# MILVLG/mmnas

Measured on AMD Instinct MI355X. Metric: supernet fwd+bwd steps/sec (VQA arch, bs=64), higher is better.
Workload: dtype f32 (bf16x6 split-operand MFMA, fp32 accumulate); 1 GPU; Net_Search supernet WEIGHT step: sample + fwd + BCE(sum) + bwd (+ gradient all-reduce), HSIZE 256, B=64/GPU, 100x2048 regions + 14 tokens, dropout 0.1 (search_vqa.py:279-292; BASELINE configs[2]); global_batch=64, parallelism=dp1, grad_allreduce=none, rccl_ranks=1, rank_id_sum_ok=True, lstm_fallback=False, dp_rows=1, dp_buckets=3, optimizer_in_step=False, gemm_split=6, hip_force_dev_kernarg=1

## Files before the change

include/mmnas_hip.h:

```cpp
#ifndef MMNAS_HIP_H
#define MMNAS_HIP_H

#include <stddef.h>
#include <stdint.h>

#ifdef __cplusplus
extern "C" {
#endif

#define MMNAS_ABI_VERSION 1

enum {
  MMNAS_OK = 0,
  MMNAS_E_SHAPE = -1,
  MMNAS_E_ARG = -2,
  MMNAS_E_LAUNCH = -3
};

enum {
  MMNAS_F_NORM = 1,
  MMNAS_F_RESIDUAL = 2,
  MMNAS_F_MASK = 4,
  MMNAS_F_REL = 8,
  MMNAS_F_SELF = 16,
// ... 156 lines not shown
size_t mmnas_rel_fused_bwd_ws_floats(int B, int Sq, int Sk);
int mmnas_rel_fused_bwd(const float* raw, const float* Wy, const float* by, const float* Wr,
                        const float* br, const float* dbiasT, float* dWy, float* dby, float* dWr,
                        float* dbr, float* ws, int B, int Sq, int Sk, int C, int R, int H,
                        void* stream);
int mmnas_rel_fused_fwd_ragged(const float* raw, const float* Wy, const float* by, const float* Wr, const float* br,
                               float* biasT, int B, int S, int C, int R, int H, const int* off, void* stream);
int mmnas_rel_fused_bwd_ragged(const float* raw, const float* Wy, const float* by, const float* Wr, const float* br,
                               const float* dbiasT, float* dWy, float* dby, float* dWr, float* dbr, float* ws,
                               int B, int S, int C, int R, int H, const int* off, const int* tile_off, int ntiles, void* stream);

#define MMNAS_REL_MULTI_MAX 32
typedef struct mmnas_rel_multi {
  int B, S, C, R, H, n_ops;
  const float* raw;
  const float* Wy; const float* by;
  float* dWy; float* dby;
  const float* Wr[MMNAS_REL_MULTI_MAX];
  const float* br[MMNAS_REL_MULTI_MAX];
  float* biasT[MMNAS_REL_MULTI_MAX];
  const float* dbiasT[MMNAS_REL_MULTI_MAX];
  float* dWr[MMNAS_REL_MULTI_MAX]; float* dbr[MMNAS_REL_MULTI_MAX];
  const int* off; const int* tile_off; int ntiles, reserved;
  float* ws;
  const unsigned char* key_mask;
} mmnas_rel_multi;
int mmnas_rel_multi_supported(int C, int R, int H);
size_t mmnas_rel_multi_bwd_ws_floats(int B, int S);
int mmnas_rel_multi_fwd(const mmnas_rel_multi* m, void* stream);
int mmnas_rel_multi_bwd(const mmnas_rel_multi* m, void* stream);
int mmnas_set_rel_hoist(int on);
int mmnas_set_rel_keylimit(int on);
int mmnas_set_guided_hoist(int on);
int mmnas_set_rel_overlap(int on);

typedef struct mmnas_mha_desc {
  int B, H, Sq, Sk, dh;
  int ldq, ldk, ldv, ldo;
  const float* Q; const float* K; const float* V;
  const uint8_t* mask;
  const float* biasT;
  float* O;
  float* lse;
  float drop_p; uint32_t drop_site; uint64_t drop_seed;
  const float* dO;
  float* dQ; float* dK; float* dV;
  float* dbiasT;
  float* delta;
  const int* q_off; const int* k_off;
} mmnas_mha_desc;

int mmnas_mha_core_fwd(const mmnas_mha_desc* d, void* stream);
int mmnas_mha_core_bwd(const mmnas_mha_desc* d, void* stream);
int mmnas_mha_core_fwd_indexed(const mmnas_mha_desc* d, const int* kv_idx, void* stream);

typedef struct mmnas_att_op {
  int B, Sq, Sk, d, di, H, dh, R;
  int flags;
  float drop_p, eps;
  uint64_t seed;
  const float* xq;
  const float* xkv;
  const uint8_t* mask;
  const float* rel;
  const float* Wq; const float* Wk; const float* Wv;
  const float* Wm;
  const float* Wr; const float* br;
  const float* ln_a; const float* ln_b;
  float* y;
  void* save;
  void* ws;
  const float* dy;
  float* dxq;
  float* dxkv;
  float* drel;
  float* dWq; float* dWk; float* dWv; float* dWm;
  float* dWr; float* dbr; float* dln_a; float* dln_b;
  int C;
  const float* Wy; const float* by;
  float* dWy; float* dby;
  const int* q_off; const int* k_off;
  int Mq, Mk;
  const int* rel_tile_off;
  int rel_ntiles, reserved2;
} mmnas_att_op;

typedef struct mmnas_plan {
  size_t save_bytes, ws_fwd_bytes, ws_bwd_bytes;
} mmnas_plan;

int mmnas_set_small_ops(int on);
int mmnas_set_small_bwd(int on);
int mmnas_set_small_ffn(int on);
int mmnas_att_op_plan(const mmnas_att_op* op, mmnas_plan* plan);
int mmnas_att_op_fwd(const mmnas_att_op* op, void* stream);
int mmnas_att_op_bwd(const mmnas_att_op* op, void* stream);

typedef struct mmnas_mlp_op {
  int M, nl;
  int dims[4];
  int flags;
  float drop_p, eps;
  uint64_t seed;
  const float* x;
  const float* W[3];
  const float* b[3];
// ... 150 lines not shown
```

mmnas_amd/_lib.py:

```python
import ctypes as C
import logging
import os

import torch

from . import switches

_HERE = os.path.dirname(os.path.abspath(__file__))
LIB_PATH = os.environ.get(switches.LIB_PATH.name) or os.path.join(_HERE, 'lib', 'libmmnas_hip.so')

log = logging.getLogger('mmnas_amd')


def _launch_configuration():
    name = 'HIP_FORCE_DEV_KERNARG'
    if name in os.environ:
        return os.environ[name], 'inherited'
    if torch.cuda.is_initialized():
        log.warning('mmnas_amd was imported after HIP had initialised and %s is not set: kernel arguments go through host-visible '
                    'memory, the ~300 short launches of a step run 20-40 %% slower.  Export %s=1 or import mmnas / mmnas_amd '
                    'before the first CUDA call.', name, name)
        return None, 'unset_after_hip_init'
    os.environ[name] = '1'
    return '1', 'set_by_library'
# ... 138 lines not shown
    'mmnas_layernorm_bwd': (_i, [_fp, _fp, _fp, _fp, _fp, _fp, _fp, _fp, _fp, _f, _u64, _u32, _i, _i, _f, _fp]),
    'mmnas_layernorm_bwd_ws_floats': (_sz, [_i, _i]),
    'mmnas_colsum': (_i, [_fp, _fp, _i, _i, _i, _fp]),
    'mmnas_eltwise_fwd': (_i, [_i, _fp, _fp, _sz, _fp]),
    'mmnas_eltwise_bwd': (_i, [_i, _fp, _fp, _fp, _sz, _fp]),
    'mmnas_drop_add': (_i, [_fp, _fp, _fp, _sz, _f, _u64, _u32, _fp]),
    'mmnas_glu_fwd': (_i, [_fp, _fp, _i, _i, _i, _f, _u64, _u32, _fp]),
    'mmnas_glu_bwd': (_i, [_fp, _fp, _fp, _i, _i, _i, _f, _u64, _u32, _fp]),
    'mmnas_rel_bias_fwd': (_i, [_fp, _fp, _fp, _fp, _i, _i, _i, _i, _i, _fp]),
    'mmnas_rel_bias_bwd': (_i, [_fp, _fp, _fp, _fp, _fp, _fp, _fp, _i, _i, _i, _i, _i, _i, _fp]),
    'mmnas_row_is_zero': (_i, [_fp, _fp, C.c_long, _i, _fp]),
    'mmnas_glimpse1_supported': (_i, [_i]),
    'mmnas_glimpse1_bwd_ws_floats': (_sz, [C.c_long, _i]),
    'mmnas_glimpse1_fwd': (_i, [_fp, _fp, _fp, _fp, C.c_long, _i, _fp]),
    'mmnas_glimpse1_bwd': (_i, [_fp, _fp, _fp, _fp, _fp, _fp, _fp, C.c_long, _i, _fp]),
    'mmnas_attflat_pool_fwd': (_i, [_fp, _fp, _fp, _fp, _fp, _i, _i, _i, _i, _fp]),
    'mmnas_attflat_pool_bwd': (_i, [_fp, _fp, _fp, _fp, _fp, _fp, _i, _i, _i, _i, _fp]),
    'mmnas_relation_embedding': (_i, [_fp, _fp, _fp, _i, _i, _fp]),
    'mmnas_semantic_embedding': (_i, [_fp, _fp, _fp, _fp, _i, _i, _i, C.c_long, _fp]),
    'mmnas_onehot_rows': (_i, [_fp, _i, _i, C.POINTER(C.c_int), _fp]),
    'mmnas_mixed_sum_ws_floats': (_sz, []),
    'mmnas_mixed_sum_fwd': (_i, [C.POINTER(_fp), _i, _fp, _fp, _sz, _fp]),
    'mmnas_mixed_sum_bwd': (_i, [C.POINTER(_fp), _i, _fp, _fp, _fp, _i, _fp, _fp, _sz, _fp]),
    'mmnas_alpha_full_step': (_i, [_fp, _fp, _fp, _fp, _fp, _i, _i, _f, _f, _f, _f, _i, _fp]),
    'mmnas_alpha_full_step_wd': (_i, [_fp, _fp, _fp, _fp, _fp, _i, _i, _f, _f, _f, _f, _f, _i, _fp]),
    'mmnas_alpha_two_step': (_i, [_fp, _fp, _fp, _fp, _fp, _i, _i, C.POINTER(C.c_int), _f, _f, _f, _f, _f, _i, _fp]),
    'mmnas_alpha_full_step_cost': (_i, [_fp] * 7 + [_i, _i, _f, _f, _f, _f, _f, _f, _f, _i, _i, _fp]),
    'mmnas_alpha_two_step_cost': (_i, [_fp] * 7 + [_i, _i, C.POINTER(C.c_int), _f, _f, _f, _f, _f, _f, _f, _i, _i, _fp]),
    'mmnas_embedding_bwd': (_i, [_fp, _fp, _fp, C.c_long, _i, C.c_long, _fp]),
    'mmnas_node_mix_fwd': (_i, [_fp, _fp, _fp, _i, _fp, _fp, _i, _i, _f, _fp]),
    'mmnas_node_mix_bwd': (_i, [_fp, _fp, _fp, _i, _fp, _fp, _fp, _i, _fp, _fp, _i, _i, _f, _fp]),
    'mmnas_node_mix_bwd_ln': (_i, [_fp, _fp, _fp, _i, _fp, _fp, _i, _fp, _fp, _fp, _fp, _fp, _fp, _fp, _fp, _f, _u64, _u32, _i, _i, _f, _fp]),
    'mmnas_embedding_bwd_det': (_i, [_fp, _fp, _fp, _fp, C.c_long, _i, C.c_long, _f, _fp]),
    'mmnas_embedding_bwd_det_ws_floats': (_sz, [C.c_long, _i]),
    'mmnas_rel_fused_supported': (_i, [_i, _i, _i]),
    'mmnas_rel_fused_fwd': (_i, [_fp, _fp, _fp, _fp, _fp, _fp, _i, _i, _i, _i, _i, _i, _fp]),
    'mmnas_rel_fused_bwd_ws_floats': (_sz, [_i, _i, _i]),
    'mmnas_rel_fused_bwd': (_i, [_fp, _fp, _fp, _fp, _fp, _fp, _fp, _fp, _fp, _fp, _fp, _i, _i, _i, _i, _i, _i, _fp]),
    'mmnas_rel_fused_fwd_ragged': (_i, [_fp, _fp, _fp, _fp, _fp, _fp, _i, _i, _i, _i, _i, _fp, _fp]),
    'mmnas_rel_fused_bwd_ragged': (_i, [_fp] * 11 + [_i, _i, _i, _i, _i, _fp, _fp, _i, _fp]),
    'mmnas_rel_multi_supported': (_i, [_i, _i, _i]),
    'mmnas_rel_multi_bwd_ws_floats': (_sz, [_i, _i]),
    'mmnas_rel_multi_fwd': (_i, [C.POINTER(RelMulti), _fp]),
    'mmnas_rel_multi_bwd': (_i, [C.POINTER(RelMulti), _fp]),
    'mmnas_set_rel_hoist': (_i, [_i]),
    'mmnas_set_rel_keylimit': (_i, [_i]),
    'mmnas_set_wgrad_live': (_i, [_i]),
    'mmnas_wgrad_live_table_ints': (_i, [_i]),
    'mmnas_wgrad_live_table': (_i, [_fp, _fp, _i, _i, _fp, _fp]),
    'mmnas_set_guided_hoist': (_i, [_i]),
    'mmnas_set_rel_overlap': (_i, [_i]),
    'mmnas_mha_core_fwd': (_i, [C.POINTER(MhaDesc), _fp]),
    'mmnas_mha_core_bwd': (_i, [C.POINTER(MhaDesc), _fp]),
    'mmnas_mha_core_fwd_indexed': (_i, [C.POINTER(MhaDesc), _fp, _fp]),
    'mmnas_itm_pair_head': (_i, [_fp] * 11 + [C.c_long, _i, _i, _f, _fp]),
    'mmnas_rank_matrix': (_i, [_fp, _i, _i, C.c_long, _fp, _fp, _fp, _fp, _fp, _fp]),
    'mmnas_row_topk': (_i, [_fp, _i, _i, C.c_long, _i, _fp, _fp, _fp]),
    'mmnas_vgd_targets': (_i, [_fp, _fp, _fp, _i, _i, C.c_double, _i, _fp, _fp, _fp, _fp, _fp, _fp, _fp]),
    'mmnas_vgd_ground': (_i, [_fp] * 5 + [_i, _i, C.c_double] + [_fp] * 7),
    'mmnas_vqa_answer': (_i, [_fp, _i, _i, C.c_long, _fp, C.c_long, _i, _i] + [_fp] * 4 + [_i] + [_fp] * 5),
    'mmnas_vqa_accuracy': (_i, [_fp] * 4 + [_i] * 4 + [_fp, _fp, _fp]),
    'mmnas_vqa_answer_targets': (_i, [_fp, _i, _i, _i, _fp, _fp, _fp]),
    'mmnas_vgd_loss_fwd': (_i, [_fp] * 6 + [_i] * 6 + [C.c_double, C.c_double] + [_fp] * 5),
    'mmnas_itm_triplet_loss_fwd': (_i, [_fp, _fp, _fp, C.c_long, _i, _f, _i, _fp, _fp, _fp]),
    'mmnas_loss_grad_scale': (_i, [_fp, _fp, _fp, _sz, _fp]),
    'mmnas_vgd_head_supported': (_i, [_i, _i]),
    'mmnas_vgd_head_bwd_ws_floats': (_sz, [_i, _i, _i]),
    'mmnas_vgd_head_fwd': (_i, [_fp] * 12 + [_i, _i, _i, _f, _i, _fp]),
    'mmnas_vgd_head_bwd': (_i, [_fp] * 20 + [_i, _i, _i, _f, _i, _fp]),
    'mmnas_att_op_plan': (_i, [C.POINTER(AttOp), C.POINTER(Plan)]),
    'mmnas_att_op_fwd': (_i, [C.POINTER(AttOp), _fp]),
    'mmnas_att_op_bwd': (_i, [C.POINTER(AttOp), _fp]),
    'mmnas_mlp_op_plan': (_i, [C.POINTER(MlpOp), C.POINTER(Plan)]),
    'mmnas_mlp_op_fwd': (_i, [C.POINTER(MlpOp), _fp]),
    'mmnas_mlp_op_bwd': (_i, [C.POINTER(MlpOp), _fp]),
    'mmnas_chain_plan': (_i, [C.POINTER(Chain), C.POINTER(C.c_size_t)]),
    'mmnas_chain_fwd': (_i, [C.POINTER(Chain), _fp]),
    'mmnas_chain_bwd': (_i, [C.POINTER(Chain), _fp]),
    'mmnas_chain_join': (_i, [_fp, _fp]),
    'mmnas_head_plan': (_i, [C.POINTER(Head), C.POINTER(C.c_size_t)]),
    'mmnas_head_fwd': (_i, [C.POINTER(Head), _fp]),
    'mmnas_head_bwd': (_i, [C.POINTER(Head), _fp]),
    'mmnas_bce_logits_sum_fwd': (_i, [_fp, _fp, _fp, _sz, _fp]),
    'mmnas_bce_logits_bwd': (_i, [_fp, _fp, _fp, _fp, _sz, _fp]),
    'mmnas_im2col_seq': (_i, [_fp, _fp, _i, _i, _i, _i, _fp]),
    'mmnas_pack_rows': (_i, [_fp, _fp, _fp, _i, _i, _i, _fp]),
    'mmnas_unpack_rows': (_i, [_fp, _fp, _fp, _i, _i, _i, _fp]),
    'mmnas_pad_seq': (_i, [_fp, _fp, _i, _i, _i, _i, _i, C.c_long, _fp]),
    'mmnas_col2im_seq': (_i, [_fp, _fp, _i, _i, _i, _i, _fp]),
    'mmnas_dwconv_seq_fwd': (_i, [_fp, _fp, _fp, _fp, _i, _i, _i, _i, _fp]),
    'mmnas_dwconv_seq_bwd': (_i, [_fp, _fp, _fp, _fp, _fp, _fp, _i, _i, _i, _i, _fp]),
    'mmnas_pack_segments': (_i, [_fp, _i, _fp, _f, _i, _fp]),
    'mmnas_pack_segments_host': (_i, [C.POINTER(Segment), _i, _fp, _f, _i, _fp]),
    'mmnas_adam_step': (_i, [_fp, _fp, _fp, _fp, _sz, _f, _f, _f, _f, _f, _fp, _f, _i, _fp]),
    'mmnas_sgd_step': (_i, [_fp, _fp, _fp, _sz, _f, _f, _f, _f, _i, _i, _fp, _f, _fp]),
    'mmnas_sumsq': (_i, [_fp, _sz, _fp, _fp]),
    'mmnas_prof_enable': (_i, [_i]),
    'mmnas_prof_collect': (_i, [C.POINTER(ProfStat)]),
}

_lib = None


class MMNasHipError(RuntimeError):
    pass

# ... 44 lines not shown
```

mmnas_amd/csrc/attention.hip:

```cpp
#include <string.h>
#include "common.h"

namespace mmnas {

struct MhaK {
  int B, H, Sq, Sk, dh, nch;
  int ldq, ldk, ldv, ldo;
  const float* Q; const float* K; const float* V;
  const uint8_t* mask; const float* biasT;
  float* O; float* stats;
  DropCfg drop; float scale;
  const float* dO; float* dQ; float* dK; float* dV; float* dbiasT; float* delta;
  const int* qoff; const int* koff;
};

template <int ROWS, int DHC, int NT>
struct TileRegs { float4 v[(ROWS * (DHC / 4) + NT - 1) / NT]; };

template <int ROWS, int DHC, int NT>
__device__ __forceinline__ void tile_fetch(TileRegs<ROWS, DHC, NT>& t, const float* __restrict__ src, int nvalid,
                                           int ld, int tid) {
  constexpr int F4 = DHC / 4, N = (ROWS * F4 + NT - 1) / NT;
#pragma unroll
  for (int i = 0; i < N; ++i) {
// ... 978 lines not shown
      if (s + 1 < NSTEP) P1(32 * ((w + s + 1) % NKB), tA[nxt], tD[nxt], tb[nxt], tm[nxt]);
      P2(k0, tA[cur], tD[cur], tb[cur], tm[cur]);
      if (s + 1 < NSTEP) {
#pragma unroll
        for (int i = 0; i < 64; ++i) {
          __builtin_amdgcn_sched_group_barrier(0x008, 1, 0);
          __builtin_amdgcn_sched_group_barrier(0x002, MMNAS_MHA_VPM, 0);
        }
      }
      P34(k0, cp, tA[cur], tD[cur]);
    }
    __syncthreads();
  }
  if (active) {
#pragma unroll
    for (int jc = 0; jc < JC; ++jc) {
      const int col = 32 * jc + l31;
#pragma unroll
      for (int r = 0; r < 16; ++r) {
        const int q = q0 + acc_row(r, hh);
        if (q < Sq) p.dQ[(qrow0 + q) * p.ldq + h * p.dh + col] = dq[jc][r];
      }
    }
  }
  for (int i = tid; i < Sk * (DHC / 4); i += 256) {
    const int key = i / (DHC / 4), c4 = i - key * (DHC / 4);
    float4 a = reinterpret_cast<const float4*>(dKs)[key * (DHC / 4) + c4];
    float4 v = reinterpret_cast<const float4*>(dVs)[key * (DHC / 4) + c4];
#pragma unroll
    for (int c = 1; c < CP; ++c) {
      const float4 a2 = reinterpret_cast<const float4*>(dKs)[(c * KB + key) * (DHC / 4) + c4];
      const float4 v2 = reinterpret_cast<const float4*>(dVs)[(c * KB + key) * (DHC / 4) + c4];
      a.x += a2.x; a.y += a2.y; a.z += a2.z; a.w += a2.w;
      v.x += v2.x; v.y += v2.y; v.z += v2.z; v.w += v2.w;
    }
    *reinterpret_cast<float4*>(p.dK + (krow0 + key) * p.ldk + h * p.dh + 4 * c4) = a;
    *reinterpret_cast<float4*>(p.dV + (krow0 + key) * p.ldv + h * p.dh + 4 * c4) = v;
  }
}


bool mha_bwd_b16_launch(int B, int H, int Sq, int Sk, int ldq, int ldk, int ldv, int ldo, const float* Q, const float* K, const float* V,
                        const float* O, const float* dO, const uint8_t* mask, const float* biasT, const float* stats, float* dQ, float* dK,
                        float* dV, float* dbiasT, DropCfg drop, float scale, const int* qoff, const int* koff, hipStream_t st);

bool mha_fwd_b16_launch(int B, int H, int Sq, int Sk, int ldq, int ldk, int ldv, int ldo, const float* Q, const float* K, const float* V,
                        const uint8_t* mask, const float* biasT, float* O, float* stats, DropCfg drop, float scale, const int* qoff,
                        const int* koff, hipStream_t st);

bool mha_fwd_b16_pair(int B, int H, int Sq, int Sk, int ld, const float* const* Q, const float* const* K, const float* const* V,
                      const uint8_t* const* mask, const float* const* biasT, float* const* O, float* const* stats, const DropCfg* drop,
                      float scale, const int* qoff, const int* koff, hipStream_t st);

static int fill(const mmnas_mha_desc* d, MhaK& k, bool bwd) {
  MMNAS_REQUIRE(d, MMNAS_E_ARG, "mha: null descriptor");
  MMNAS_REQUIRE(d->B > 0 && d->H > 0 && d->Sq > 0 && d->Sk > 0, MMNAS_E_SHAPE, "mha: B=%d H=%d Sq=%d Sk=%d", d->B,
                d->H, d->Sq, d->Sk);
  MMNAS_REQUIRE(d->dh == 16 || d->dh == 32 || d->dh == 64 || d->dh == 128 || d->dh == 256, MMNAS_E_SHAPE,
                "mha: head dim %d not in {16,32,64,128,256}", d->dh);
  MMNAS_REQUIRE(d->Q && d->K && d->V && d->lse, MMNAS_E_ARG, "mha: null Q/K/V/stats");
  MMNAS_REQUIRE(d->ldq % 4 == 0 && d->ldk % 4 == 0 && d->ldv % 4 == 0 && d->ldo % 4 == 0, MMNAS_E_SHAPE,
                "mha: row strides must be multiples of 4 floats");
  MMNAS_REQUIRE((((uintptr_t)d->Q | (uintptr_t)d->K | (uintptr_t)d->V) & 15) == 0, MMNAS_E_ARG,
                "mha: Q/K/V must be 16-byte aligned");
  MMNAS_REQUIRE((double)d->B * d->H * d->Sq * d->Sk < 4294967296.0, MMNAS_E_SHAPE, "mha: score tensor too large");
  k.B = d->B; k.H = d->H; k.Sq = d->Sq; k.Sk = d->Sk; k.dh = d->dh;
  k.ldq = d->ldq; k.ldk = d->ldk; k.ldv = d->ldv; k.ldo = d->ldo;
  k.Q = d->Q; k.K = d->K; k.V = d->V; k.mask = d->mask; k.biasT = d->biasT; k.O = d->O; k.stats = d->lse;
  k.drop = make_drop(d->drop_p, d->drop_seed, d->drop_site);
  k.scale = 1.0f / sqrtf((float)d->dh);
  k.dO = d->dO; k.dQ = d->dQ; k.dK = d->dK; k.dV = d->dV; k.dbiasT = d->dbiasT; k.delta = d->delta;
  k.qoff = d->q_off; k.koff = d->k_off;
  if (k.qoff || k.koff) {
    MMNAS_REQUIRE(d->dh == 64 && d->Sq <= 128 && d->Sk <= 128, MMNAS_E_SHAPE, "mha: packed rows (q_off / k_off) need d_h = 64 and at most 128 queries / keys per sequence (Sq=%d Sk=%d dh=%d)", d->Sq, d->Sk, d->dh);
    MMNAS_REQUIRE(!(k.koff && d->mask), MMNAS_E_ARG, "mha: packed keys carry no padding: no mask with k_off");
  }
  if (bwd) {
    MMNAS_REQUIRE(d->dO && d->dQ && d->dK && d->dV && d->delta && d->O, MMNAS_E_ARG, "mha_bwd: null gradient buffer");
    MMNAS_REQUIRE((((uintptr_t)d->dO | (uintptr_t)d->O) & 15) == 0, MMNAS_E_ARG, "mha_bwd: dO/O alignment");
  } else {
    MMNAS_REQUIRE(d->O, MMNAS_E_ARG, "mha_fwd: null output");
  }
  return MMNAS_OK;
}

static int mha_nw() { return sw::mha_nw.get() == 2 ? 2 : 4; }

static int mha_stream_mink() {
  const int v = sw::mha_stream_mink.get();
  return v < 1 ? 1 : v > 257 ? 257 : v;
}
static bool mha_streams(const MhaK& k) { return !k.qoff && !k.koff && k.Sk >= mha_stream_mink(); }

static void launch_fwd_stream(const MhaK& k, hipStream_t st) {
  const dim3 grid(cdiv(k.Sq, 128), k.H, k.B), block(256);
  switch (k.dh) {
    case 16: MMNAS_LAUNCH((mha_fwd_stream_kernel<16, 1, 1>), grid, block, 0, st, k); break;
    case 32: MMNAS_LAUNCH((mha_fwd_stream_kernel<32, 1, 1>), grid, block, 0, st, k); break;
    case 64: MMNAS_LAUNCH((mha_fwd_stream_kernel<64, 1, 1>), grid, block, 0, st, k); break;
    case 128: MMNAS_LAUNCH((mha_fwd_stream_kernel<64, 2, 2>), grid, block, 0, st, k); break;
    default: MMNAS_LAUNCH((mha_fwd_stream_kernel<64, 4, 2>), dim3(grid.x, 2 * k.H, k.B), block, 0, st, k); break;
  }
}

template <int DHC>
static void launch_fwd(const MhaK& k, hipStream_t st) {
// ... 38 lines not shown
  const bool on = sw::mha_pair.get() != 0;
  const int nkc = cdiv(k0.Sk, 32);
  const bool same = on && k0.B == k1.B && k0.H == k1.H && k0.Sq == k1.Sq && k0.Sk == k1.Sk && k0.dh == 64 && k1.dh == 64 &&
                    nkc > 2 && nkc <= 4 && k0.Sq > 64 && mha_nw() == 4 && !k0.qoff == !k1.qoff && !k0.koff == !k1.koff &&
                    !mha_streams(k0) && !mha_streams(k1);
  if (!same) {
    if ((rc = mmnas_mha_core_fwd(d0, st))) return rc;
    return mmnas_mha_core_fwd(d1, st);
  }
  k0.nch = k1.nch = 1;
  const double bhqk = (double)k0.B * k0.H * k0.Sq * k0.Sk;
  if (k0.ldq == k0.ldk && k0.ldq == k0.ldv && k0.ldq == k0.ldo && k1.ldq == k0.ldq && k1.ldk == k0.ldq && k1.ldv == k0.ldq && k1.ldo == k0.ldq &&
      k0.qoff == k1.qoff && k0.koff == k1.koff) {
    const float* Qs[2] = {k0.Q, k1.Q}; const float* Ks[2] = {k0.K, k1.K}; const float* Vs[2] = {k0.V, k1.V};
    const uint8_t* Ms[2] = {k0.mask, k1.mask}; const float* Bs[2] = {k0.biasT, k1.biasT};
    float* Os[2] = {k0.O, k1.O}; float* Ss[2] = {k0.stats, k1.stats};
    const DropCfg Ds[2] = {k0.drop, k1.drop};
    ProfScope ps16(MMNAS_K_MHA_FWD, 8.0 * bhqk * k0.dh,
                   4.0 * (2.0 * (double)k0.B * k0.H * k0.dh * (2.0 * k0.Sq + 2.0 * k0.Sk) + (k0.biasT ? bhqk : 0.0) + (k1.biasT ? bhqk : 0.0)), st);
    if (mha_fwd_b16_pair(k0.B, k0.H, k0.Sq, k0.Sk, k0.ldq, Qs, Ks, Vs, Ms, Bs, Os, Ss, Ds, k0.scale, k0.qoff, k0.koff, st))
      return check_launch("mha_core_fwd_pair");
  }
  ProfScope ps(MMNAS_K_MHA_FWD, 8.0 * bhqk * k0.dh,
               4.0 * (2.0 * (double)k0.B * k0.H * k0.dh * (2.0 * k0.Sq + 2.0 * k0.Sk) + (k0.biasT ? bhqk : 0.0) + (k1.biasT ? bhqk : 0.0)), st);
  const int nqb = cdiv(k0.Sq, 128);
  MMNAS_LAUNCH((mha_fwd_pair_kernel<64, 4, 4>), dim3(2 * nqb, k0.H, k0.B), dim3(256), 0, st, k0, k1, nqb);
  return check_launch("mha_core_fwd_pair");
}

template <int DHC>
static void launch_fwd_idx(const MhaK& k, const int* kv_idx, hipStream_t st) {
  const int nkc = cdiv(k.Sk, 32);
#define FWDI(NKC, NW) MMNAS_LAUNCH((mha_fwd_idx_kernel<DHC, NKC, NW>), dim3(cdiv(k.Sq, 32 * NW), k.H, k.B), \
                                   dim3(64 * NW), 0, st, k, kv_idx)
  const int nwmax = mha_nw();
  if (k.Sq <= 32) { if (nkc <= 1) FWDI(1, 1); else FWDI(2, 1); }
  else if (k.Sq <= 64 || nwmax == 2) { if (nkc <= 1) FWDI(1, 2); else FWDI(2, 2); }
  else { if (nkc <= 1) FWDI(1, 4); else FWDI(2, 4); }
#undef FWDI
}

int mha_core_fwd_indexed(const mmnas_mha_desc* d, const int* kv_idx, hipStream_t st) {
  MhaK k;
  int rc = fill(d, k, false);
  if (rc) return rc;
  MMNAS_REQUIRE(kv_idx, MMNAS_E_ARG, "mha_indexed: null kv_idx");
  MMNAS_REQUIRE(d->Sk <= 64, MMNAS_E_SHAPE, "mha_indexed: Sk=%d keys; the indexed core serves at most 64 keys", d->Sk);
  MMNAS_REQUIRE(d->B <= 65535, MMNAS_E_SHAPE, "mha_indexed: B=%d query batches; at most 65535 per call", d->B);
  MMNAS_REQUIRE(d->drop_p == 0.f, MMNAS_E_ARG, "mha_indexed: drop_p=%g; the indexed core has no dropout", d->drop_p);
  MMNAS_REQUIRE(!d->biasT, MMNAS_E_ARG, "mha_indexed: the indexed core has no score bias (biasT must be NULL)");
  MMNAS_REQUIRE(!d->q_off && !d->k_off, MMNAS_E_ARG, "mha_indexed: the indexed core has no packed rows (q_off / k_off must be NULL)");
  const double bhqk = (double)k.B * k.H * k.Sq * k.Sk;
  ProfScope ps(MMNAS_K_MHA_FWD, 4.0 * bhqk * k.dh, 4.0 * ((double)k.B * k.H * k.dh * (2.0 * k.Sq + 2.0 * k.Sk)), st);
  if (k.dh >= 64) { k.nch = k.dh / 64; launch_fwd_idx<64>(k, kv_idx, st); }
  else if (k.dh == 32) { k.nch = 1; launch_fwd_idx<32>(k, kv_idx, st); }
  else { k.nch = 1; launch_fwd_idx<16>(k, kv_idx, st); }
  return check_launch("mha_core_fwd_indexed");
}

}

using namespace mmnas;

extern "C" int mmnas_mha_core_fwd(const mmnas_mha_desc* d, void* stream) {
  MhaK k;
  int rc = fill(d, k, false);
  if (rc) return rc;
  hipStream_t st = (hipStream_t)stream;
  const double bhqk = (double)k.B * k.H * k.Sq * k.Sk;
  ProfScope ps(MMNAS_K_MHA_FWD, 4.0 * bhqk * k.dh,
               4.0 * ((double)k.B * k.H * k.dh * (2.0 * k.Sq + 2.0 * k.Sk) + (k.biasT ? bhqk : 0.0)), st);
  if (mha_streams(k)) { k.nch = k.dh >= 64 ? k.dh / 64 : 1; launch_fwd_stream(k, st); return check_launch("mha_core_fwd"); }
  if (k.dh == 64 && mha_fwd_b16_launch(k.B, k.H, k.Sq, k.Sk, k.ldq, k.ldk, k.ldv, k.ldo, k.Q, k.K, k.V, k.mask, k.biasT, k.O, k.stats,
                                       k.drop, k.scale, k.qoff, k.koff, st))
    return check_launch("mha_core_fwd");
  if (k.dh >= 64) { k.nch = k.dh / 64; launch_fwd<64>(k, st); }
  else if (k.dh == 32) { k.nch = 1; launch_fwd<32>(k, st); }
  else { k.nch = 1; launch_fwd<16>(k, st); }
  return check_launch("mha_core_fwd");
}

extern "C" int mmnas_mha_core_bwd(const mmnas_mha_desc* d, void* stream) {
  MhaK k;
  int rc = fill(d, k, true);
  if (rc) return rc;
  hipStream_t st = (hipStream_t)stream;
  const double bhqk = (double)k.B * k.H * k.Sq * k.Sk;
  ProfScope ps(MMNAS_K_MHA_BWD, 10.0 * bhqk * k.dh,
               4.0 * ((double)k.B * k.H * k.dh * (4.0 * k.Sq + 4.0 * k.Sk) + (k.biasT ? 2.0 * bhqk : 0.0)), st);
  const bool fused_on = sw::mha_bwd_fused.get() != 0;
  const bool packed = k.qoff || k.koff;
  if (packed) MMNAS_REQUIRE((((uintptr_t)k.dK | (uintptr_t)k.dV) & 15) == 0, MMNAS_E_ARG, "mha_bwd: dK / dV alignment (packed rows run the fused kernel only)");
  if ((fused_on || packed) && k.dh == 64 && k.Sq <= 128 && k.Sk <= 128 && (((uintptr_t)k.dK | (uintptr_t)k.dV) & 15) == 0) {
    k.nch = 1;
    if (mha_bwd_b16_launch(k.B, k.H, k.Sq, k.Sk, k.ldq, k.ldk, k.ldv, k.ldo, k.Q, k.K, k.V, (const float*)d->O, k.dO, k.mask, k.biasT,
                           k.stats, k.dQ, k.dK, k.dV, k.dbiasT, k.drop, k.scale, k.qoff, k.koff, st))
      return check_launch("mha_core_bwd");
    const dim3 grid(k.H, k.B);
    const int nkb = cdiv(k.Sk, 32);
    if (k.dbiasT) {
      if (nkb <= 1) MMNAS_LAUNCH((mha_bwd_fused_kernel<1, true>), grid, dim3(256), 0, st, k);
      else if (nkb <= 2) MMNAS_LAUNCH((mha_bwd_fused_kernel<2, true>), grid, dim3(256), 0, st, k);
      else MMNAS_LAUNCH((mha_bwd_fused_kernel<4, true>), grid, dim3(256), 0, st, k);
    } else {
      if (nkb <= 1) MMNAS_LAUNCH((mha_bwd_fused_kernel<1, false>), grid, dim3(256), 0, st, k);
      else if (nkb <= 2) MMNAS_LAUNCH((mha_bwd_fused_kernel<2, false>), grid, dim3(256), 0, st, k);
      else MMNAS_LAUNCH((mha_bwd_fused_kernel<4, false>), grid, dim3(256), 0, st, k);
    }
    return check_launch("mha_core_bwd");
  }
  if (k.dh > 64) {
    const long n = (long)k.B * k.Sq * k.H;
    int blocks = (int)((n + 255) / 256);
    if (blocks > 2048) blocks = 2048;
    MMNAS_LAUNCH(mha_delta_kernel, dim3(blocks), dim3(256), 0, st, k.dO, (const float*)d->O, k.delta, k.B, k.H,
                       k.Sq, k.dh, k.ldo);
  }
  if (k.dh >= 64) { k.nch = k.dh / 64; launch_bwd<64>(k, st); }
  else if (k.dh == 32) { k.nch = 1; launch_bwd<32>(k, st); }
  else { k.nch = 1; launch_bwd<16>(k, st); }
  return check_launch("mha_core_bwd");
}
```

mmnas_amd/csrc/switches.h:

```cpp
#pragma once

namespace mmnas {

int env_int(const char* name, int dflt);

enum SwKind { sw_int, sw_bool, sw_exact1, sw_presence, sw_string };
enum SwPolicy { sw_once, sw_every_call, sw_reload };

struct Switch {
  const char* name;
  int dflt;
  SwKind kind;
  SwPolicy policy;
  const char* help;
  int value;
  int state;

  int get() { return state ? value : read(); }
  int read();
  int reload();
  int set(int v);
  int peek(int* source) const;
};

#define MMNAS_SWITCHES(X) \
   \
  X(chain_overlap, "MMNAS_CHAIN_OVERLAP", 0, bool, once, "language stream beside the leading image-stream operators (mmnas_set_chain_overlap); measured: no gain, DESIGN.md section 5") \
  X(head_overlap, "MMNAS_HEAD_OVERLAP", 0, bool, once, "the answer head's two AttFlat sides on two streams") \
  X(head_glimpse1, "MMNAS_HEAD_GLIMPSE1", 1, bool, every_call, "0: the head's one-glimpse logit layer as GEMM launches (A/B, tests); ops.py reads it too") \
  X(head_projt, "MMNAS_HEAD_PROJT", 1, bool, every_call, "0: the answer projection's gradients from the untransposed loss gradient") \
  X(rel_hoist, "MMNAS_REL_HOIST", 1, bool, once, "relation bias of all lazy-handle operators of a stream in one launch per direction (mmnas_set_rel_hoist); 0: one fused launch per operator (supernet step 4.54 -> 5.00 ms)") \
  X(rel_overlap, "MMNAS_REL_OVERLAP", 0, bool, once, "the image stream's relation launches on a second stream (mmnas_set_rel_overlap); measured slower, +2.5 % on the supernet step") \
  X(node_lnb, "MMNAS_NODE_LNB", 1, bool, once, "architecture step: the sampled candidate's LayerNorm backward inside the node's mix kernel (7.81 -> 7.72 ms, profiles/r06_node_lnb_ab.txt); 0: its own launch") \
  X(guided_hoist, "MMNAS_GUIDED_HOIST", 1, bool, once, "key / value projections of a chain's guided operators as grouped launches (mmnas_set_guided_hoist)") \
  X(rel_fwd_valu, "MMNAS_REL_FWD_VALU", 0, exact1, every_call, "1: a lone RelSelfAtt computes its bias with the per-operator fused kernel instead of the one-operator multi kernel (A/B)") \
  X(side_prio, "MMNAS_SIDE_PRIO", 1, bool, every_call, "0: the chains' extra streams without stream priorities (read when a stream pair is created)") \
  X(side_flush, "MMNAS_SIDE_FLUSH", 0, string, once, "op: side-stream parameter-gradient work released behind every operator instead of once per phase") \
  X(wgrad_live, "MMNAS_WGRAD_LIVE", 1, int, once, "image-stream weight gradients of a padded batch's chain reduce over the 32-row K-tiles that cover the live gradient rows only (mmnas_set_wgrad_live); 0: all B Sy rows") \
   \
  X(small_ops, "MMNAS_SMALL_OPS", 1, bool, once, "SelfAtt of <= 16 rows as one launch forward (mmnas_set_small_ops); 0: the general path") \
  X(small_bwd, "MMNAS_SMALL_BWD", 1, bool, once, "the same operators' backward as two launches (mmnas_set_small_bwd)") \
  X(small_ffn, "MMNAS_SMALL_FFN", 0, int, once, "FeedForward forward as one launch (mmnas_set_small_ffn): 1 four slices of 256 hidden units, 2 eight of 128; measured neutral (profiles/r05_small_ffn_ab.txt)") \
   \
  X(gemm_ln, "MMNAS_GEMM_LN", 0, exact1, once, "1: the merge / last FFN product and its LayerNorm as one row-panel launch (mmnas_set_gemm_ln); measured neutral, profiles/r06_ab.txt") \
  X(gemm_ln_minm, "MMNAS_GEMM_LN_MINM", 2048, int, once, "fewest rows for the row-panel kernel (read together with MMNAS_GEMM_LN)") \
  X(gemm_ln_maxk, "MMNAS_GEMM_LN_MAXK", 256, int, once, "largest K for the row-panel kernel (read together with MMNAS_GEMM_LN)") \
   \
  X(mha_nw, "MMNAS_MHA_NW", 4, int, every_call, "2: attention cores never use 4-wave workgroups (4-wave groups measured 7-15 % faster; the streaming forward always runs four)") \
  X(mha_stream_mink, "MMNAS_MHA_STREAM_MINK", 257, int, every_call, "fewest keys at which the attention forward streams the keys in blocks of 128 (1..257; more than 256 keys always stream; dense rows only)") \
  X(mha_pair, "MMNAS_MHA_PAIR", 1, bool, once, "0: two attention cores of one geometry as two launches (mixed chain)") \
  X(mha_bwd_fused, "MMNAS_MHA_BWD_FUSED", 1, bool, once, "0: the attention backward as separate dQ and dK / dV kernels (dense rows only)") \
  X(mha_fwd_b16, "MMNAS_MHA_FWD_B16", 1, bool, once, "0: attention forward (d_h = 64, 65..128 keys) on the fp32 MFMA kernels instead of split-bf16 operands (profiles/r06_attention_b16_ab.txt)") \
  X(mha_fwd_b16_two, "MMNAS_MHA_FWD_B16_TWO", 320, int, once, "more than this many (sample, head) pairs: the split-bf16 forward runs two per workgroup") \
  X(mha_bwd_b16, "MMNAS_MHA_BWD_B16", 1, bool, once, "0: attention backward (d_h = 64, 65..128 keys) on the fp32 MFMA kernels instead of split-bf16 operands (supernet step -1.6 % with both)") \
   \
  X(rel_multi_dbg, "MMNAS_REL_MULTI_DBG", 0, int, once, "timing experiments of a -DMMNAS_DBG_REL=1 build only (wrong results): 1 no stores, 2 no raw reloads, 4 no head-projection MFMAs") \
  X(rel_multi_wgs, "MMNAS_REL_MULTI_WGS", 3, int, once, "workgroups per CU of the multi-operator relation forward (tuning)") \
  X(rel_multi_yield, "MMNAS_REL_MULTI_YIELD", 0, int, once, "1 | 3: the multi-operator relation kernels' yield variants (tuning)") \
  X(rel_keylimit, "MMNAS_REL_KEYLIMIT", 1, int, once, "multi-operator relation kernels of a padded batch walk only the elements under keys up to each sample's last unmasked one (mmnas_set_rel_keylimit); 0: all B S^2 elements") \
  X(rel_bwd_valu, "MMNAS_REL_BWD_VALU", 1, bool, once, "0: the fused relation backward as the all-MFMA kernel (A/B)") \
   \
  X(gemm_tile, "MMNAS_GEMM_TILE", 0, int, reload, "64 | 128: force the tile shape") \
  X(gemm_generic, "MMNAS_GEMM_GENERIC", 0, presence, reload, "set (to anything): force the guarded-load path; ops.py reads it too") \
  X(gemm_sk, "MMNAS_GEMM_SK", 1, int, reload, "stream-K / split-K: 0 never, 1 automatic, 2 always") \
  X(gemm_wgs, "MMNAS_GEMM_WGS", 0, int, reload, "co-resident workgroup budget (0: 1024 for 64^2 tiles, 512 for 128^2)") \
  X(gemm_min_units, "MMNAS_GEMM_MIN_UNITS", 4, int, reload, "fewest K-tiles a workgroup is given (at least 1)") \
  X(gemm_gm, "MMNAS_GEMM_GM", 0, int, reload, "row-panels per tile-order block (0: 8)") \
  X(gemm_xcd, "MMNAS_GEMM_XCD", 1, int, reload, "0: identity workgroup mapping") \
  X(gemm_split, "MMNAS_GEMM_SPLIT", 6, int, reload, "products as 6 / 3 / 1 bf16 MFMA products of split operands (6: fp32-grade; 3, 1: reduced precision), 0: fp32 MFMA") \
  X(gemm_pair, "MMNAS_GEMM_PAIR", 1, int, reload, "0: mmnas_gemm_pair launches its two products separately") \
  X(gemm_split_slots, "MMNAS_GEMM_SPLIT_SLOTS", 0, int, reload, "split-K pieces wanted over all tiles (0: from SPLIT_P and SPLIT_MINWG)") \
  X(gemm_split_p, "MMNAS_GEMM_SPLIT_P", 24, int, reload, "K-tiles per split-K piece (at least 1)") \
  X(gemm_split_minwg, "MMNAS_GEMM_SPLIT_MINWG", 256, int, reload, "fewest split-K pieces in total when pieces of SPLIT_P would be fewer") \
  X(gemm_pf, "MMNAS_GEMM_PF", 2, int, reload, "1 | 2: K-tiles of operand loads in flight ahead of the MFMA block (64^2 fp32 path)") \
  X(gemm_hyb_t, "MMNAS_GEMM_HYB_T", 16, int, reload, "fewest K-tiles per output tile for the whole-tiles + streamed-tail hybrid") \
  X(gemm_lean, "MMNAS_GEMM_LEAN", 3, int, reload, "lean kernels: bit 0 NT / NN products, bit 1 split-K TN products") \
  X(gemm_lean_maxb, "MMNAS_GEMM_LEAN_MAXB", 8 << 20, int, reload, "largest B matrix (bytes) the lean tile order is used for") \
  X(lstm_fwd_p, "MMNAS_LSTM_FWD_P", 0, int, every_call, "K-tiles per workgroup of the LSTM forward step's stream-K product (0: whole tiles; read per time step)") \
  X(lstm_bwd_p, "MMNAS_LSTM_BWD_P", 8, int, every_call, "K-tiles per workgroup of the LSTM backward step's stream-K product (0: whole tiles; read per time step)") \
   \
  X(prof_dump, "MMNAS_PROF_DUMP", 0, string, every_call, "file: mmnas_prof_collect appends one kind,tag,ms,flops,bytes row per bracketed launch (tools/prof_shapes.py)")

namespace sw {
#define MMNAS_SW_DECLARE(id, var, dflt, kind, policy, help) extern Switch id;
MMNAS_SWITCHES(MMNAS_SW_DECLARE)
#undef MMNAS_SW_DECLARE
}

}
```

Before: 233.0 steps/s.

## Add 16-key attention kernels for short-key guided attention backward

Adds dedicated MFMA kernels for attention cores with at most 16 keys and d_h 64, the case of guided operators attending to the 14 question tokens. By default only the backward path uses them. The new kernel handles one (sample, head) per workgroup with waves striding over query tiles, keeps K/V in registers, and reduces dK/dV across waves in shared memory. The aim is to avoid padding these shapes to 32-key chunks in the generic kernels, at the cost of a new code path that must match the existing dropout and mask semantics.

Result: no change. 234.6 steps/s, median of 6 (+0.7%).

```diff
diff --git a/include/mmnas_hip.h b/include/mmnas_hip.h
--- a/include/mmnas_hip.h
+++ b/include/mmnas_hip.h
@@ -232,6 +232,8 @@
 
 int mmnas_mha_core_fwd(const mmnas_mha_desc* d, void* stream);
 int mmnas_mha_core_bwd(const mmnas_mha_desc* d, void* stream);
+int mmnas_set_mha_sk16(int mode);
+int mmnas_mha_sk16_serves(const mmnas_mha_desc* d, int bwd);
 int mmnas_mha_core_fwd_indexed(const mmnas_mha_desc* d, const int* kv_idx, void* stream);
 
 typedef struct mmnas_att_op {
diff --git a/mmnas_amd/_lib.py b/mmnas_amd/_lib.py
--- a/mmnas_amd/_lib.py
+++ b/mmnas_amd/_lib.py
@@ -214,6 +214,8 @@
     'mmnas_set_rel_overlap': (_i, [_i]),
     'mmnas_mha_core_fwd': (_i, [C.POINTER(MhaDesc), _fp]),
     'mmnas_mha_core_bwd': (_i, [C.POINTER(MhaDesc), _fp]),
+    'mmnas_set_mha_sk16': (_i, [_i]),
+    'mmnas_mha_sk16_serves': (_i, [C.POINTER(MhaDesc), _i]),
     'mmnas_mha_core_fwd_indexed': (_i, [C.POINTER(MhaDesc), _fp, _fp]),
     'mmnas_itm_pair_head': (_i, [_fp] * 11 + [C.c_long, _i, _i, _f, _fp]),
     'mmnas_rank_matrix': (_i, [_fp, _i, _i, C.c_long, _fp, _fp, _fp, _fp, _fp, _fp]),
diff --git a/mmnas_amd/csrc/attention.hip b/mmnas_amd/csrc/attention.hip
--- a/mmnas_amd/csrc/attention.hip
+++ b/mmnas_amd/csrc/attention.hip
@@ -1054,6 +1054,10 @@
                       const uint8_t* const* mask, const float* const* biasT, float* const* O, float* const* stats, const DropCfg* drop,
                       float scale, const int* qoff, const int* koff, hipStream_t st);
 
+bool mha_sk16_serves(const mmnas_mha_desc* d, bool bwd);
+void mha_sk16_fwd_launch(const mmnas_mha_desc* d, DropCfg drop, float scale, hipStream_t st, const int* kvidx = nullptr);
+void mha_sk16_bwd_launch(const mmnas_mha_desc* d, DropCfg drop, float scale, hipStream_t st);
+
 static int fill(const mmnas_mha_desc* d, MhaK& k, bool bwd) {
   MMNAS_REQUIRE(d, MMNAS_E_ARG, "mha: null descriptor");
   MMNAS_REQUIRE(d->B > 0 && d->H > 0 && d->Sq > 0 && d->Sk > 0, MMNAS_E_SHAPE, "mha: B=%d H=%d Sq=%d Sk=%d", d->B,
@@ -1198,6 +1202,7 @@
   MMNAS_REQUIRE(!d->q_off && !d->k_off, MMNAS_E_ARG, "mha_indexed: the indexed core has no packed rows (q_off / k_off must be NULL)");
   const double bhqk = (double)k.B * k.H * k.Sq * k.Sk;
   ProfScope ps(MMNAS_K_MHA_FWD, 4.0 * bhqk * k.dh, 4.0 * ((double)k.B * k.H * k.dh * (2.0 * k.Sq + 2.0 * k.Sk)), st);
+  if (mha_sk16_serves(d, false)) { mha_sk16_fwd_launch(d, k.drop, k.scale, st, kv_idx); return check_launch("mha_core_fwd_indexed"); }
   if (k.dh >= 64) { k.nch = k.dh / 64; launch_fwd_idx<64>(k, kv_idx, st); }
   else if (k.dh == 32) { k.nch = 1; launch_fwd_idx<32>(k, kv_idx, st); }
   else { k.nch = 1; launch_fwd_idx<16>(k, kv_idx, st); }
@@ -1217,6 +1222,7 @@
   ProfScope ps(MMNAS_K_MHA_FWD, 4.0 * bhqk * k.dh,
                4.0 * ((double)k.B * k.H * k.dh * (2.0 * k.Sq + 2.0 * k.Sk) + (k.biasT ? bhqk : 0.0)), st);
   if (mha_streams(k)) { k.nch = k.dh >= 64 ? k.dh / 64 : 1; launch_fwd_stream(k, st); return check_launch("mha_core_fwd"); }
+  if (mha_sk16_serves(d, false)) { mha_sk16_fwd_launch(d, k.drop, k.scale, st); return check_launch("mha_core_fwd"); }
   if (k.dh == 64 && mha_fwd_b16_launch(k.B, k.H, k.Sq, k.Sk, k.ldq, k.ldk, k.ldv, k.ldo, k.Q, k.K, k.V, k.mask, k.biasT, k.O, k.stats,
                                        k.drop, k.scale, k.qoff, k.koff, st))
     return check_launch("mha_core_fwd");
@@ -1237,6 +1243,7 @@
   const bool fused_on = sw::mha_bwd_fused.get() != 0;
   const bool packed = k.qoff || k.koff;
   if (packed) MMNAS_REQUIRE((((uintptr_t)k.dK | (uintptr_t)k.dV) & 15) == 0, MMNAS_E_ARG, "mha_bwd: dK / dV alignment (packed rows run the fused kernel only)");
+  if (mha_sk16_serves(d, true)) { mha_sk16_bwd_launch(d, k.drop, k.scale, st); return check_launch("mha_core_bwd"); }
   if ((fused_on || packed) && k.dh == 64 && k.Sq <= 128 && k.Sk <= 128 && (((uintptr_t)k.dK | (uintptr_t)k.dV) & 15) == 0) {
     k.nch = 1;
     if (mha_bwd_b16_launch(k.B, k.H, k.Sq, k.Sk, k.ldq, k.ldk, k.ldv, k.ldo, k.Q, k.K, k.V, (const float*)d->O, k.dO, k.mask, k.biasT,
diff --git a/mmnas_amd/csrc/attention_sk16.hip b/mmnas_amd/csrc/attention_sk16.hip
--- /dev/null
+++ b/mmnas_amd/csrc/attention_sk16.hip
@@ -0,0 +1,289 @@
+#include "common.h"
+
+namespace mmnas {
+
+struct MhaSk16K {
+  int B, H, Sq, Sk;
+  int ldq, ldk, ldv, ldo;
+  const float* Q; const float* K; const float* V; const uint8_t* mask;
+  float* O; float* stats;
+  const float* dO; float* dQ; float* dK; float* dV;
+  DropCfg drop; float scale;
+};
+
+__device__ __forceinline__ f32x4 sk16_mfma(float a, float b, f32x4 c) {
+  return __builtin_amdgcn_mfma_f32_16x16x4f32(a, b, c, 0, 0, 0);
+}
+#define SK16_MFMA4(ACC, AF, BF)        \
+  ACC = sk16_mfma(AF.x, BF.x, ACC);    \
+  ACC = sk16_mfma(AF.y, BF.y, ACC);    \
+  ACC = sk16_mfma(AF.z, BF.z, ACC);    \
+  ACC = sk16_mfma(AF.w, BF.w, ACC);
+
+__device__ __forceinline__ float4 sk16_ld4(const float* ptr, bool ok) {
+  const float4 x = *reinterpret_cast<const float4*>(ptr);
+  return ok ? x : make_float4(0.f, 0.f, 0.f, 0.f);
+}
+
+template <bool IDX>
+__global__ void __launch_bounds__(256) mha_sk16_fwd_kernel(const MhaSk16K p, const int* __restrict__ kvidx) {
+  const int tid = threadIdx.x, lane = tid & 63, w = tid >> 6, l15 = lane & 15, kq = lane >> 4;
+  const int b = blockIdx.z, h = blockIdx.y, q0 = 64 * blockIdx.x + 16 * w;
+  const int Sq = p.Sq, Sk = p.Sk;
+  if (q0 >= Sq) return;
+  const size_t bh = (size_t)b * p.H + h, krow0 = (size_t)(IDX ? kvidx[b] : b) * Sk;
+  const int qi = q0 + l15;
+  const bool qok = qi < Sq, kok = l15 < Sk;
+
+  const float* krow = p.K + (krow0 + (kok ? l15 : 0)) * p.ldk + h * 64 + 4 * kq;
+  const float* qrow = p.Q + ((size_t)b * Sq + (qok ? qi : Sq - 1)) * p.ldq + h * 64 + 4 * kq;
+  float4 kf[4], qf[4];
+#pragma unroll
+  for (int s = 0; s < 4; ++s) {
+    kf[s] = sk16_ld4(krow + 16 * s, kok);
+    qf[s] = *reinterpret_cast<const float4*>(qrow + 16 * s);
+  }
+  float vb[4][4];
+#pragma unroll
+  for (int r = 0; r < 4; ++r) {
+    const int key = 4 * kq + r;
+    const bool ok = key < Sk;
+    const float* vrow = p.V + (krow0 + (ok ? key : 0)) * p.ldv + h * 64 + l15;
+#pragma unroll
+    for (int jt = 0; jt < 4; ++jt) {
+      const float x = vrow[16 * jt];
+      vb[r][jt] = ok ? x : 0.f;
+    }
+  }
+  const bool mk = p.mask ? (kok && p.mask[krow0 + (kok ? l15 : 0)] != 0) : false;
+  const unsigned mbits = (unsigned)__ballot(mk) & 0xffffu;
+
+  f32x4 acc = {0.f, 0.f, 0.f, 0.f};
+#pragma unroll
+  for (int s = 0; s < 4; ++s) { SK16_MFMA4(acc, kf[s], qf[s]) }
+
+  float m = -INFINITY;
+#pragma unroll
+  for (int r = 0; r < 4; ++r) {
+    const int key = 4 * kq + r;
+    float v = acc[r] * p.scale;
+    v = ((mbits >> key) & 1u) ? -1e9f : v;
+    v = key < Sk ? v : -INFINITY;
+    acc[r] = v;
+    m = fmaxf(m, v);
+  }
+  m = fmaxf(m, __shfl_xor(m, 16, 64));
+  m = fmaxf(m, __shfl_xor(m, 32, 64));
+  float sum = 0.f;
+#pragma unroll
+  for (int r = 0; r < 4; ++r) {
+    const float e = __expf(acc[r] - m);
+    acc[r] = e;
+    sum += e;
+  }
+  sum += __shfl_xor(sum, 16, 64);
+  sum += __shfl_xor(sum, 32, 64);
+  const float inv = 1.0f / sum;
+  if (qok && kq == 0) {
+    p.stats[(bh * Sq + qi) * 2] = m;
+    p.stats[(bh * Sq + qi) * 2 + 1] = inv;
+  }
+  const uint32_t dpre = drop_pre(p.drop, (uint32_t)((bh * Sq + qi) * Sk + 4 * kq));
+#pragma unroll
+  for (int r = 0; r < 4; ++r) {
+    float a = acc[r] * inv;
+    if (p.drop.thresh) a *= drop_mult_pre(p.drop, dpre + (uint32_t)r * DROP_G);
+    acc[r] = a;
+  }
+
+  float* orow = p.O + ((size_t)b * Sq + (qok ? qi : 0)) * p.ldo + h * 64 + 4 * kq;
+#pragma unroll
+  for (int jt = 0; jt < 4; ++jt) {
+    f32x4 o = {0.f, 0.f, 0.f, 0.f};
+#pragma unroll
+    for (int r = 0; r < 4; ++r) o = sk16_mfma(vb[r][jt], acc[r], o);
+    if (qok) *reinterpret_cast<float4*>(orow + 16 * jt) = make_float4(o[0], o[1], o[2], o[3]);
+  }
+}
+
+constexpr int SK16_PLD = 68;
+constexpr int SK16_TLD = 20;
+
+template <int NW>
+__global__ void __launch_bounds__(64 * NW) mha_sk16_bwd_kernel(const MhaSk16K p) {
+  __shared__ __attribute__((aligned(16))) float part[NW][2][16 * SK16_PLD];
+  __shared__ __attribute__((aligned(16))) float TrAll[NW][16 * SK16_TLD];
+  const int tid = threadIdx.x, lane = tid & 63, w = tid >> 6, l15 = lane & 15, kq = lane >> 4;
+  const int h = blockIdx.x, b = blockIdx.y;
+  const int Sq = p.Sq, Sk = p.Sk;
+  const size_t bh = (size_t)b * p.H + h, krow0 = (size_t)b * Sk, qrow0 = (size_t)b * Sq;
+  const bool kok = l15 < Sk;
+  float* Tr = TrAll[w];
+
+  const float* krow = p.K + (krow0 + (kok ? l15 : 0)) * p.ldk + h * 64 + 4 * kq;
+  const float* vrow = p.V + (krow0 + (kok ? l15 : 0)) * p.ldv + h * 64 + 4 * kq;
+  float4 kf[4], vf[4];
+#pragma unroll
+  for (int s = 0; s < 4; ++s) {
+    kf[s] = sk16_ld4(krow + 16 * s, kok);
+    vf[s] = sk16_ld4(vrow + 16 * s, kok);
+  }
+  float kb[4][4];
+#pragma unroll
+  for (int c = 0; c < 4; ++c) {
+    const int key = 4 * kq + c;
+    const bool ok = key < Sk;
+    const float* kr = p.K + (krow0 + (ok ? key : 0)) * p.ldk + h * 64 + l15;
+#pragma unroll
+    for (int jt = 0; jt < 4; ++jt) {
+      const float x = kr[16 * jt];
+      kb[c][jt] = ok ? x : 0.f;
+    }
+  }
+  const bool masked = p.mask ? (kok && p.mask[krow0 + (kok ? l15 : 0)] != 0) : false;
+
+  f32x4 dk[4], dv[4];
+#pragma unroll
+  for (int jt = 0; jt < 4; ++jt) { dk[jt] = (f32x4){0.f, 0.f, 0.f, 0.f}; dv[jt] = (f32x4){0.f, 0.f, 0.f, 0.f}; }
+
+  const int ntiles = (Sq + 15) >> 4;
+  for (int t = w; t < ntiles; t += NW) {
+    const int q0 = 16 * t;
+    const int qi = q0 + l15;
+    const bool qok = qi < Sq;
+    const size_t row = qrow0 + (qok ? qi : Sq - 1);
+    const float* qrow = p.Q + row * p.ldq + h * 64 + 4 * kq;
+    const float* grow = p.dO + row * p.ldo + h * 64 + 4 * kq;
+    const float* orow = p.O + row * p.ldo + h * 64 + 4 * kq;
+    float4 qf[4], gf[4], of[4];
+#pragma unroll
+    for (int s = 0; s < 4; ++s) {
+      qf[s] = *reinterpret_cast<const float4*>(qrow + 16 * s);
+      gf[s] = *reinterpret_cast<const float4*>(grow + 16 * s);
+      of[s] = *reinterpret_cast<const float4*>(orow + 16 * s);
+    }
+    float4 qb[4], gb[4];
+    float mr[4], ir[4];
+#pragma unroll
+    for (int r = 0; r < 4; ++r) {
+      const int q = q0 + 4 * kq + r;
+      const bool ok = q < Sq;
+      const size_t rr = qrow0 + (ok ? q : Sq - 1);
+      qb[r] = sk16_ld4(p.Q + rr * p.ldq + h * 64 + 4 * l15, ok);
+      gb[r] = sk16_ld4(p.dO + rr * p.ldo + h * 64 + 4 * l15, ok);
+      const float sm = p.stats[(bh * Sq + (ok ? q : Sq - 1)) * 2], si = p.stats[(bh * Sq + (ok ? q : Sq - 1)) * 2 + 1];
+      mr[r] = ok ? sm : 0.f;
+      ir[r] = ok ? si : 0.f;
+    }
+    float del = 0.f;
+#pragma unroll
+    for (int s = 0; s < 4; ++s) del += (gf[s].x * of[s].x + gf[s].y * of[s].y) + (gf[s].z * of[s].z + gf[s].w * of[s].w);
+    del += __shfl_xor(del, 16, 64);
+    del += __shfl_xor(del, 32, 64);
+
+    f32x4 sc = {0.f, 0.f, 0.f, 0.f}, da = {0.f, 0.f, 0.f, 0.f};
+#pragma unroll
+    for (int s = 0; s < 4; ++s) {
+      SK16_MFMA4(sc, qf[s], kf[s])
+      SK16_MFMA4(da, gf[s], vf[s])
+    }
+    const uint32_t dpre = drop_pre(p.drop, (uint32_t)((bh * Sq + q0 + 4 * kq) * Sk + l15));
+#pragma unroll
+    for (int r = 0; r < 4; ++r) {
+      const bool ok = kok && q0 + 4 * kq + r < Sq;
+      const float dl = __shfl(del, 4 * kq + r, 64);
+      float v = sc[r] * p.scale;
+      v = masked ? -1e9f : v;
+      const float pr = __expf(v - mr[r]) * ir[r];
+      const float dm = drop_mult_pre(p.drop, dpre + (uint32_t)(r * Sk) * DROP_G);
+      const float dz = (ok && !masked) ? pr * (da[r] * dm - dl) : 0.f;
+      sc[r] = dz * p.scale;
+      da[r] = ok ? pr * dm : 0.f;
+    }
+#pragma unroll
+    for (int r = 0; r < 4; ++r) {
+      dk[0] = sk16_mfma(qb[r].x, sc[r], dk[0]); dk[1] = sk16_mfma(qb[r].y, sc[r], dk[1]);
+      dk[2] = sk16_mfma(qb[r].z, sc[r], dk[2]); dk[3] = sk16_mfma(qb[r].w, sc[r], dk[3]);
+      dv[0] = sk16_mfma(gb[r].x, da[r], dv[0]); dv[1] = sk16_mfma(gb[r].y, da[r], dv[1]);
+      dv[2] = sk16_mfma(gb[r].z, da[r], dv[2]); dv[3] = sk16_mfma(gb[r].w, da[r], dv[3]);
+    }
+#pragma unroll
+    for (int r = 0; r < 4; ++r) Tr[(4 * kq + r) * SK16_TLD + l15] = sc[r];
+    __builtin_amdgcn_wave_barrier();
+    const f32x4 tz = *reinterpret_cast<const f32x4*>(Tr + l15 * SK16_TLD + 4 * kq);
+    __builtin_amdgcn_wave_barrier();
+    float* dqrow = p.dQ + (qrow0 + (qok ? qi : 0)) * p.ldq + h * 64 + 4 * kq;
+#pragma unroll
+    for (int jt = 0; jt < 4; ++jt) {
+      f32x4 dq = {0.f, 0.f, 0.f, 0.f};
+#pragma unroll
+      for (int c = 0; c < 4; ++c) dq = sk16_mfma(kb[c][jt], tz[c], dq);
+      if (qok) *reinterpret_cast<float4*>(dqrow + 16 * jt) = make_float4(dq[0], dq[1], dq[2], dq[3]);
+    }
+  }
+
+#pragma unroll
+  for (int r = 0; r < 4; ++r) {
+    const int o = l15 * SK16_PLD + 16 * kq + 4 * r;
+    *reinterpret_cast<float4*>(part[w][0] + o) = make_float4(dk[0][r], dk[1][r], dk[2][r], dk[3][r]);
+    *reinterpret_cast<float4*>(part[w][1] + o) = make_float4(dv[0][r], dv[1][r], dv[2][r], dv[3][r]);
+  }
+  __syncthreads();
+  for (int i = tid; i < 2 * 16 * 16; i += 64 * NW) {
+    const int which = i >> 8, key = (i >> 4) & 15, c4 = i & 15;
+    if (key >= Sk) continue;
+    float4 a = *reinterpret_cast<const float4*>(part[0][which] + key * SK16_PLD + 4 * c4);
+#pragma unroll
+    for (int x = 1; x < NW; ++x) {
+      const float4 a2 = *reinterpret_cast<const float4*>(part[x][which] + key * SK16_PLD + 4 * c4);
+      a.x += a2.x; a.y += a2.y; a.z += a2.z; a.w += a2.w;
+    }
+    float* dst = which ? p.dV + (krow0 + key) * p.ldv : p.dK + (krow0 + key) * p.ldk;
+    *reinterpret_cast<float4*>(dst + h * 64 + 4 * c4) = a;
+  }
+}
+
+bool mha_sk16_serves(const mmnas_mha_desc* d, bool bwd) {
+  const int mode = sw::mha_sk16.get();
+  if (bwd ? mode == 0 : mode != 1) return false;
+  if (d->dh != 64 || d->Sk > 16 || d->biasT || d->q_off || d->k_off || d->B > 65535 || d->H > 65535) return false;
+  if (bwd) {
+    if (d->dbiasT || !sw::mha_bwd_fused.get()) return false;
+    return (((uintptr_t)d->dQ | (uintptr_t)d->dK | (uintptr_t)d->dV | (uintptr_t)d->dO | (uintptr_t)d->O) & 15) == 0;
+  }
+  return ((uintptr_t)d->O & 15) == 0;
+}
+
+static MhaSk16K sk16_fill(const mmnas_mha_desc* d, DropCfg drop, float scale) {
+  MhaSk16K k;
+  k.B = d->B; k.H = d->H; k.Sq = d->Sq; k.Sk = d->Sk;
+  k.ldq = d->ldq; k.ldk = d->ldk; k.ldv = d->ldv; k.ldo = d->ldo;
+  k.Q = d->Q; k.K = d->K; k.V = d->V; k.mask = d->mask; k.O = d->O; k.stats = d->lse;
+  k.dO = d->dO; k.dQ = d->dQ; k.dK = d->dK; k.dV = d->dV;
+  k.drop = drop; k.scale = scale;
+  return k;
+}
+
+void mha_sk16_fwd_launch(const mmnas_mha_desc* d, DropCfg drop, float scale, hipStream_t st, const int* kvidx) {
+  const MhaSk16K k = sk16_fill(d, drop, scale);
+  const dim3 grid(cdiv(k.Sq, 64), k.H, k.B);
+  if (kvidx) MMNAS_LAUNCH((mha_sk16_fwd_kernel<true>), grid, dim3(256), 0, st, k, kvidx);
+  else MMNAS_LAUNCH((mha_sk16_fwd_kernel<false>), grid, dim3(256), 0, st, k, kvidx);
+}
+
+void mha_sk16_bwd_launch(const mmnas_mha_desc* d, DropCfg drop, float scale, hipStream_t st) {
+  const MhaSk16K k = sk16_fill(d, drop, scale);
+  const dim3 grid(k.H, k.B);
+  const int ntiles = cdiv(k.Sq, 16);
+  if (ntiles <= 1) MMNAS_LAUNCH((mha_sk16_bwd_kernel<1>), grid, dim3(64), 0, st, k);
+  else if (ntiles <= 2) MMNAS_LAUNCH((mha_sk16_bwd_kernel<2>), grid, dim3(128), 0, st, k);
+  else if (ntiles <= 4) MMNAS_LAUNCH((mha_sk16_bwd_kernel<4>), grid, dim3(256), 0, st, k);
+  else MMNAS_LAUNCH((mha_sk16_bwd_kernel<8>), grid, dim3(512), 0, st, k);
+}
+
+}
+
+using namespace mmnas;
+
+extern "C" int mmnas_set_mha_sk16(int mode) { return sw::mha_sk16.set(mode < 0 ? 0 : mode > 2 ? 2 : mode); }
+extern "C" int mmnas_mha_sk16_serves(const mmnas_mha_desc* d, int bwd) { return d && mha_sk16_serves(d, bwd != 0) ? 1 : 0; }
diff --git a/mmnas_amd/csrc/switches.h b/mmnas_amd/csrc/switches.h
--- a/mmnas_amd/csrc/switches.h
+++ b/mmnas_amd/csrc/switches.h
@@ -53,6 +53,7 @@
   X(mha_fwd_b16, "MMNAS_MHA_FWD_B16", 1, bool, once, "0: attention forward (d_h = 64, 65..128 keys) on the fp32 MFMA kernels instead of split-bf16 operands (profiles/r06_attention_b16_ab.txt)") \
   X(mha_fwd_b16_two, "MMNAS_MHA_FWD_B16_TWO", 320, int, once, "more than this many (sample, head) pairs: the split-bf16 forward runs two per workgroup") \
   X(mha_bwd_b16, "MMNAS_MHA_BWD_B16", 1, bool, once, "0: attention backward (d_h = 64, 65..128 keys) on the fp32 MFMA kernels instead of split-bf16 operands (supernet step -1.6 % with both)") \
+  X(mha_sk16, "MMNAS_MHA_SK16", 2, int, once, "attention cores of at most 16 keys (d_h = 64, dense rows, no bias: the guided operators) on the 16-row kernels of attention_sk16.hip (mmnas_set_mha_sk16): 2 the backward only, 1 forward and backward, 0 the 32-key-chunk kernels") \
    \
   X(rel_multi_dbg, "MMNAS_REL_MULTI_DBG", 0, int, once, "timing experiments of a -DMMNAS_DBG_REL=1 build only (wrong results): 1 no stores, 2 no raw reloads, 4 no head-projection MFMAs") \
   X(rel_multi_wgs, "MMNAS_REL_MULTI_WGS", 3, int, once, "workgroups per CU of the multi-operator relation forward (tuning)") \
```
